# XuZhang1211/PVPUFormer

Hardware: AMD Instinct MI355X
Metric: 448x448 images/sec fwd+bwd, ViT-B VPUFormer (higher is better)
Workload: dtype bf16

## Files before the change

### include/vpu_hip.h

```cpp
#ifndef VPU_HIP_H
#define VPU_HIP_H
#include <stdint.h>

#ifdef __cplusplus
extern "C" {
#endif

#define VPU_BF16 0
#define VPU_F32 1

#define VPU_EPI_BIAS 1
#define VPU_EPI_PREACT 2
#define VPU_EPI_GELU 4
#define VPU_EPI_RELU 8
#define VPU_EPI_DGELU 16
#define VPU_EPI_DRELU 32
#define VPU_EPI_RESID 64
#define VPU_EPI_AFFINE 128
#define VPU_EPI_ACCUM 256
#define VPU_EPI_OUT_F32 512
#define VPU_EPI_SAVE_DGELU 1024
#define VPU_EPI_MULAUX 2048

typedef struct vpu_gemm_desc {
// ... 192 lines not shown
int vpu_groupnorm_nchunk(void);
int vpu_groupnorm_fwd(const void* x, const float* w, const float* b, void* y, float* mean, float* rstd, double* stats,
                      int32_t B, int64_t HW, int32_t C, float eps, int32_t gelu, int32_t dtype, void* stream);
int vpu_groupnorm_bwd(const void* dy, const void* x, const float* w, const float* b, const float* mean,
                      const float* rstd, void* dx, float* part, double* stats, int32_t B, int64_t HW, int32_t C,
                      int32_t gelu, int32_t dtype, void* stream);
int vpu_bilinear_cl_fwd(const void* in, int32_t ld_in, void* out, int32_t ld_out, int32_t B, int32_t h, int32_t w,
                        int32_t H, int32_t W, int32_t C, int32_t dtype, void* stream);
int vpu_bilinear_cl_bwd(const void* dout, int32_t ld_out, void* din, int32_t ld_in, int32_t B, int32_t h, int32_t w,
                        int32_t H, int32_t W, int32_t C, int32_t dtype, void* stream);
int vpu_upsum_relu(void* io, const void* const* z, const int32_t* h, const int32_t* w, int32_t n, int32_t B, int32_t H,
                   int32_t W, int32_t C, int32_t dtype, void* stream);
int vpu_head_grad_fused(const void* dfn, const void* y, const float* inv, const float* dout, const void* x, const float* w,
                        const float* mask, void* dx, float* part, float* part_b, int64_t rows, int64_t HW, int32_t C,
                        int32_t dtype, void* stream);
int vpu_gate_stats(const void* Q, const void* Kt, float* cg, int32_t* argq, float* sg, int32_t* argc, int32_t B,
                   int32_t nq, int32_t N, int32_t C, int32_t dtype, void* stream);
int vpu_gate_apply(const void* x, const float* cg, const float* sg, void* out, int32_t B, int32_t N, int32_t C,
                   int32_t dtype, void* stream);
int vpu_gate_bwd(const void* dout, const void* x, const float* cg, const int32_t* argq, const float* sg,
                 const int32_t* argc, void* dx, int32_t accum, void* dQ, void* dK, float* part, int32_t B, int32_t nq,
                 int32_t N, int32_t C, int32_t dtype, void* stream);
int vpu_gate_fwd_n(const void* const* Q, const void* const* K, const void* x, void* const* out, float* cg, int32_t* argq,
                   float* sg, int32_t* argc, int32_t n, int32_t B, int32_t nq, int32_t N, int32_t C, int32_t dtype, void* stream);
int vpu_gate_bwd_n(const void* const* dout, const void* x, const float* cg, const int32_t* argq, const float* sg,
                   const int32_t* argc, void* dx, int32_t accum, void* const* dQ, void* const* dK, float* part, int32_t n,
                   int32_t B, int32_t nq, int32_t N, int32_t C, int32_t dtype, void* stream);
int vpu_convseg_fwd(const void* x, const float* w, const float* bias, const float* mask, float* out, int64_t rows,
                    int64_t HW, int32_t C, int32_t dtype, void* stream);
int vpu_convseg_bwd_nblk(int64_t rows);
// ... 36 lines not shown
```

### pvpuformer_amd/_lib.py

```python
import ctypes as C
import os

_HERE = os.path.dirname(os.path.abspath(__file__))
LIB_PATH = os.path.join(_HERE, os.environ.get("VPU_LIB_FILE") or
                        ("libvpu_hip_diag.so" if os.environ.get("VPU_LIB_DIAG", "0") == "1" else "libvpu_hip.so"))

BF16, F32 = 0, 1

EPI_BIAS, EPI_PREACT, EPI_GELU, EPI_RELU, EPI_DGELU, EPI_DRELU = 1, 2, 4, 8, 16, 32
EPI_RESID, EPI_AFFINE, EPI_ACCUM, EPI_OUT_F32 = 64, 128, 256, 512
EPI_SAVE_DGELU, EPI_MULAUX = 1024, 2048


class GemmDesc(C.Structure):
    _fields_ = [
        ("A", C.c_void_p), ("B", C.c_void_p), ("C", C.c_void_p), ("bias", C.c_void_p), ("resid", C.c_void_p),
        ("aux", C.c_void_p), ("preact", C.c_void_p),
        ("M", C.c_int32), ("N", C.c_int32), ("K", C.c_int32),
        ("lda", C.c_int32), ("ldb", C.c_int32), ("ldc", C.c_int32), ("ldr", C.c_int32), ("ldaux", C.c_int32),
        ("batch", C.c_int32), ("inner", C.c_int32),
        ("sAo", C.c_int64), ("sAi", C.c_int64), ("sBo", C.c_int64), ("sBi", C.c_int64),
        ("sCo", C.c_int64), ("sCi", C.c_int64), ("sRo", C.c_int64), ("sRi", C.c_int64),
        ("transA", C.c_int32), ("transB", C.c_int32), ("dtype", C.c_int32), ("flags", C.c_int32),
        ("resid_period", C.c_int32),
# ... 92 lines not shown
    "vpu_patch_im2col_floor": [_P, _P, _P, _I, _I, _I, _I, _I, _I, _I, _P],
    "vpu_window_permute": [_P, _P, _I, _I, _I, _I, _I, _I, _P],
    "vpu_space_to_depth2_crop": [_P, _P, _I, _I, _I, _I, _I, _P],
    "vpu_pixel_shuffle2": [_P, _P, _P, _I, _I, _I, _I, _I, _I, _P],
    "vpu_pixel_shuffle2_gn_stats": [_P, _P, _P, _P, _I, _I, _I, _I, _I, _P],
    "vpu_groupnorm_apply": [_P, _P, _P, _P, _P, _P, _P, _I, _L, _I, _F, _I, _I, _P],
    "vpu_pixel_unshuffle2_nblk": [_I],
    "vpu_pixel_unshuffle2_sums": [_P, _P, _P, _I, _I, _I, _I, _I, _P],
    "vpu_groupnorm_nchunk": [],
    "vpu_groupnorm_fwd": [_P, _P, _P, _P, _P, _P, _P, _I, _L, _I, _F, _I, _I, _P],
    "vpu_groupnorm_bwd": [_P, _P, _P, _P, _P, _P, _P, _P, _P, _I, _L, _I, _I, _I, _P],
    "vpu_bilinear_cl_fwd": [_P, _I, _P, _I, _I, _I, _I, _I, _I, _I, _I, _P],
    "vpu_bilinear_cl_bwd": [_P, _I, _P, _I, _I, _I, _I, _I, _I, _I, _I, _P],
    "vpu_head_grad_fused": [_P, _P, _P, _P, _P, _P, _P, _P, _P, _P, _L, _L, _I, _I, _P],
    "vpu_upsum_relu": [_P, C.POINTER(C.c_void_p), C.POINTER(C.c_int32), C.POINTER(C.c_int32), _I, _I, _I, _I, _I, _I, _P],
    "vpu_gate_stats": [_P, _P, _P, _P, _P, _P, _I, _I, _I, _I, _I, _P],
    "vpu_gate_apply": [_P, _P, _P, _P, _I, _I, _I, _I, _P],
    "vpu_gate_bwd": [_P, _P, _P, _P, _P, _P, _P, _I, _P, _P, _P, _I, _I, _I, _I, _I, _P],
    "vpu_gate_fwd_n": [C.POINTER(C.c_void_p), C.POINTER(C.c_void_p), _P, C.POINTER(C.c_void_p), _P, _P, _P, _P, _I, _I, _I, _I, _I, _I, _P],
    "vpu_gate_bwd_n": [C.POINTER(C.c_void_p), _P, _P, _P, _P, _P, _P, _I, C.POINTER(C.c_void_p), C.POINTER(C.c_void_p), _P, _I, _I, _I,
                       _I, _I, _I, _P],
    "vpu_convseg_fwd": [_P, _P, _P, _P, _P, _L, _L, _I, _I, _P],
    "vpu_convseg_bwd_nblk": [_L],
    "vpu_convseg_bwd": [_P, _P, _P, _P, _P, _I, _P, _P, _L, _L, _I, _I, _P],
    "vpu_upsample_ac_fwd": [_P, _P, _L, _I, _I, _I, _I, _P],
    "vpu_upsample_ac_bwd": [_P, _P, _L, _I, _I, _I, _I, _P],
    "vpu_p2cl_fwd_bwd": [_P, _P, _P, _P, _P, _P, _F, _I, _I, _I, _I, _P],
    "vpu_p2cl_up_nband": [_I, _I],
    "vpu_p2cl_up_fwd_bwd": [_P, _P, _P, _P, _P, _P, _F, _I, _I, _I, _I, _I, _I, _P],
    "vpu_nfl_dice_scratch_doubles": [_I],
# ... 47 lines not shown
```

### pvpuformer_amd/csrc/spatial.hip

```cpp
#include <stdlib.h>
#include "vpu_common.h"
#include "interp_ac.h"
#include "../../include/vpu_hip.h"

#define DISPATCH_T(dtype, ...)                                   \
    if ((dtype) == VPU_BF16) { using T = bf16_t; __VA_ARGS__ }   \
    else if ((dtype) == VPU_F32) { using T = float; __VA_ARGS__ } \
    else { vpu_set_error("bad dtype"); return VPU_ERR_ARG; }
#define ST reinterpret_cast<hipStream_t>(stream)

namespace {

__constant__ float c_mean[3] = {0.485f, 0.456f, 0.406f};
__constant__ float c_std[3] = {0.229f, 0.224f, 0.225f};

template <typename T, bool NORM = true, bool VEC = true>
__global__ __launch_bounds__(256) void patch_im2col_kernel(const float* __restrict__ img4,
                                                           const float* __restrict__ disks, T* __restrict__ cols,
                                                           int B, int H, int W, int P, int wg) {
    const int gw = W / P, gh = H / P;
    const int K3 = 3 * P * P, K3P = (K3 + 7) / 8 * 8;
    const int Tn = gw * gh, KK = 2 * K3P, chunks = KK / 8;
    const int64_t total = (int64_t)B * Tn * chunks;
    const int nwx = gw / wg;
// ... 503 lines not shown
                const int64_t base = (int64_t)b * h * w;
                load8(in + (base + (int64_t)y0 * w + x0) * C + ck * 8, p);
                load8(in + (base + (int64_t)y0 * w + x1) * C + ck * 8, q);
                load8(in + (base + (int64_t)y1 * w + x0) * C + ck * 8, r);
                load8(in + (base + (int64_t)y1 * w + x1) * C + ck * 8, s);
#pragma unroll
                for (int j = 0; j < 8; ++j) o[j] += hy * (hx * p[j] + lx * q[j]) + ly * (hx * r[j] + lx * s[j]);
            }
#pragma unroll
        for (int j = 0; j < 8; ++j) o[j] = fmaxf(o[j], 0.f);
        store8(io + pix * C + ck * 8, o);
    }
}

template <typename T>
__global__ __launch_bounds__(256) void upsum_relu2_kernel(T* __restrict__ io, const UpsumArgs a, int B, int H, int W, int C) {
    const int chunks = C / 8, H2 = H >> 1, W2 = W >> 1;
    const int64_t total = (int64_t)B * H2 * W2 * chunks;
    for (int64_t i = (int64_t)blockIdx.x * 256 + threadIdx.x; i < total; i += (int64_t)gridDim.x * 256) {
        const int ck = (int)(i % chunks);
        const int64_t blk = i / chunks;
        const int X = 2 * (int)(blk % W2), Y = 2 * (int)((blk / W2) % H2), b = (int)(blk / ((int64_t)W2 * H2));
        float o[2][2][8];
#pragma unroll
        for (int dy = 0; dy < 2; ++dy)
#pragma unroll
            for (int dx = 0; dx < 2; ++dx) load8(io + (((int64_t)b * H + Y + dy) * W + X + dx) * C + ck * 8, o[dy][dx]);
#pragma unroll
        for (int m = 0; m < 3; ++m)
            if (m < a.n) {
                const int h = a.h[m], w = a.w[m];
                const T* __restrict__ in = reinterpret_cast<const T*>(a.z[m]) + (int64_t)b * h * w * C + ck * 8;
                int y0a, y1a, y0b, y1b, x0a, x1a, x0b, x1b;
                float lya, lyb, lxa, lxb;
                src_index_half(Y, (float)h / (float)H, h, y0a, y1a, lya);
                src_index_half(Y + 1, (float)h / (float)H, h, y0b, y1b, lyb);
                src_index_half(X, (float)w / (float)W, w, x0a, x1a, lxa);
                src_index_half(X + 1, (float)w / (float)W, w, x0b, x1b, lxb);
                const bool sy = y0b != y0a, sx = x0b != x0a;
                const int ry[3] = {y0a, y1a, y1b}, rx[3] = {x0a, x1a, x1b};
                float ha[3][8], hb[3][8];
#pragma unroll
                for (int r = 0; r < 3; ++r) {
                    if (r == 2 && !sy) continue;
                    float t0[8], t1[8], t2[8];
                    load8(in + ((int64_t)ry[r] * w + rx[0]) * C, t0);
                    load8(in + ((int64_t)ry[r] * w + rx[1]) * C, t1);
                    if (sx) load8(in + ((int64_t)ry[r] * w + rx[2]) * C, t2);
#pragma unroll
                    for (int j = 0; j < 8; ++j) {
                        ha[r][j] = (1.f - lxa) * t0[j] + lxa * t1[j];
                        const float u0 = sx ? t1[j] : t0[j], u1 = sx ? t2[j] : t1[j];
                        hb[r][j] = (1.f - lxb) * u0 + lxb * u1;
                    }
                }
#pragma unroll
                for (int j = 0; j < 8; ++j) {
                    o[0][0][j] += (1.f - lya) * ha[0][j] + lya * ha[1][j];
                    o[0][1][j] += (1.f - lya) * hb[0][j] + lya * hb[1][j];
                    const float a0 = sy ? ha[1][j] : ha[0][j], a1 = sy ? ha[2][j] : ha[1][j];
                    const float b0 = sy ? hb[1][j] : hb[0][j], b1 = sy ? hb[2][j] : hb[1][j];
                    o[1][0][j] += (1.f - lyb) * a0 + lyb * a1;
                    o[1][1][j] += (1.f - lyb) * b0 + lyb * b1;
                }
            }
#pragma unroll
        for (int dy = 0; dy < 2; ++dy)
#pragma unroll
            for (int dx = 0; dx < 2; ++dx) {
#pragma unroll
                for (int j = 0; j < 8; ++j) o[dy][dx][j] = fmaxf(o[dy][dx][j], 0.f);
                store8(io + (((int64_t)b * H + Y + dy) * W + X + dx) * C + ck * 8, o[dy][dx]);
            }
    }
}

template <typename T>
__global__ __launch_bounds__(256) void bilinear_cl_bwd_kernel(const T* __restrict__ dout, int ld_out,
                                                              T* __restrict__ din, int ld_in, int B, int h, int w, int H,
                                                              int W, int C) {
    const int chunks = C / 8;
    const float sh = (float)h / (float)H, sw = (float)w / (float)W;
    const float fh = (float)H / (float)h, fw = (float)W / (float)w;
    const int64_t total = (int64_t)B * h * w * chunks;
    for (int64_t i = (int64_t)blockIdx.x * 256 + threadIdx.x; i < total; i += (int64_t)gridDim.x * 256) {
        const int ck = (int)(i % chunks);
        const int64_t pix = i / chunks;
// ... 951 lines not shown
    a.n = n;
    for (int i = 0; i < 3; ++i) {
        a.z[i] = i < n ? z[i] : nullptr; a.h[i] = i < n ? h[i] : 1; a.w[i] = i < n ? w[i] : 1;
        if (i < n && (!z[i] || h[i] < 1 || w[i] < 1)) { vpu_set_error("upsum_relu: null / empty map"); return VPU_ERR_ARG; }
    }
    const int64_t total = (int64_t)B * H * W * (C / 8);
    bool quad = n > 0 && H % 2 == 0 && W % 2 == 0;
    for (int i = 0; i < n; ++i) quad = quad && H % h[i] == 0 && W % w[i] == 0 && H / h[i] >= 2 && W / w[i] >= 2;
    if (quad) {
        DISPATCH_T(dtype, upsum_relu2_kernel<T><<<vpu_grid_for(total / 4, 256, 16384), 256, 0, ST>>>((T*)io, a, B, H, W, C);)
    } else {
        DISPATCH_T(dtype, upsum_relu_kernel<T><<<vpu_grid_for(total, 256, 16384), 256, 0, ST>>>((T*)io, a, B, H, W, C);)
    }
    return vpu_check_launch("vpu_upsum_relu");
}
extern "C" int vpu_bilinear_cl_bwd(const void* dout, int32_t ld_out, void* din, int32_t ld_in, int32_t B, int32_t h,
                                   int32_t w, int32_t H, int32_t W, int32_t C, int32_t dtype, void* stream) {
    vpu_clear_stale_error();
    if (C % 8 || ld_in % 8 || ld_out % 8) { vpu_set_error("bilinear_cl_bwd: C, ld % 8"); return VPU_ERR_ARG; }
    const int64_t total = (int64_t)B * h * w * (C / 8);
    const int R = (h > 0 && w > 0 && H % h == 0 && W % w == 0 && H / h == W / w) ? H / h : 0;
    static const int split_min = [] { const char* e = vpu_lab_getenv("VPU_BILINEAR_SPLIT_R"); return e ? atoi(e) : 8; }();
    if ((R == 4 || R == 8) && R >= split_min && C == 256) {
        const unsigned g2 = (unsigned)(8 * ((((int64_t)B * h * w + 1) / 2 + 7) / 8));
        DISPATCH_T(dtype,
                   if (R == 4) bilinear_cl_bwd_int4_kernel<T, 4><<<g2, 256, 0, ST>>>((const T*)dout, ld_out, (T*)din, ld_in, B, h, w);
                   else bilinear_cl_bwd_int4_kernel<T, 8><<<g2, 256, 0, ST>>>((const T*)dout, ld_out, (T*)din, ld_in, B, h, w);)
        return vpu_check_launch("vpu_bilinear_cl_bwd");
    }
    if (R == 2 || R == 4 || R == 8) {
// ... 158 lines not shown
```

### pvpuformer_amd/engine.py

```python
import contextlib
import math
import os
from collections import OrderedDict
from types import SimpleNamespace

import numpy as np
import torch

from . import ops
from ._lib import (BF16, F32, EPI_BIAS, EPI_PREACT, EPI_GELU, EPI_RELU, EPI_DGELU, EPI_DRELU, EPI_RESID, EPI_AFFINE,
                   EPI_ACCUM, EPI_OUT_F32, EPI_SAVE_DGELU, EPI_MULAUX)


class Tape:
    __slots__ = ("fns", "out_grads", "done", "sim_low", "lane")

    def __init__(self):
        self.fns = []
        self.out_grads = [None, None, None]
        self.done = False
        self.sim_low = None
        self.lane = None

    def append(self, fn):
# ... 97 lines not shown
        self.wgrad_fill = 0.8
        hid = self.D * c["mlp_ratio"]
        blk = sum(((n + 255) // 256) * ((k + 127) // 128) for n, k in ((3 * self.D, self.D), (self.D, self.D), (hid, self.D), (self.D, hid)))
        pk = os.environ.get("VPU_WGRAD_PACK", "")
        k3 = ops.gemm_get_option("k3")
        k4_default = (k3 & 8) != 0
        self.pack_wgrad = pk == "1" or (pk != "0" and (blk < 0.95 * 256 or k4_default))
        self.k3_wgrad = (k3 & 1) != 0
        self.k4_wgrad = (k3 & 8) != 0
        self.wgrad_round = 256 if (self.k4_wgrad or not self.k3_wgrad) else 512
        self.wgrad_tn = 256 if self.k4_wgrad else 128
        self.unify_wgrad = True
        self.lazy_zero = True
        self.xattn_split = max(1, int(os.environ.get("VPU_XATTN_SPLIT", "1")))
        self.neck_lanes = int(os.environ.get("VPU_NECK_LANES", "0"))
        self._tok_stream = None
        self._in_lanes = False
        self.dist_colsum = True
        self._pack_seen, self._pack_total = {}, {}
        self._pending_reports, self._reporting = [], False
        self.group_tiles = 256
        self.split_wgrad = True
        self._wq = []
        self._csq = []
        self._gq = []
        self._gq_out = set()
        self._frozen = set()
        self._token_rows = 0
        self.grad_ready_hook = None
        self.report_lag = max(1, int(os.environ.get("VPU_DIST_REPORT_LAG", "2")))
# ... 983 lines not shown
        gf = self.G("head.fusion_conv.conv.weight")
        relu_done, ymask = [False], [[False] for _ in range(4)]
        ys, zs = [], []
        for i in range(4):
            f, s = feats[i]
            ys.append(self.linear(f, f"head.convs.{i}.conv.weight", f"head.convs.{i}.conv.bias", B * s * s, Cc, o[i],
                                  act="relu", pre_masked=ymask[i]))
        fused = Var(self._new(B * HW4, Cc))
        ops.gemm(ys[0].t, wf, fused.t, B * HW4, Cc, Cc, Cc, ldf, Cc, self.dt, flags=EPI_BIAS,
                 bias=self.Pm("head.fusion_conv.conv.bias"))
        for i in (1, 2, 3):
            s = feats[i][1]
            z = self._new(B * s * s, Cc)
            ops.gemm(ys[i].t, (wf[0], wf[1] + i * Cc), z, B * s * s, Cc, Cc, Cc, ldf, Cc, self.dt)
            zs.append((z, s, s))
        ops.upsum_relu(fused.t, zs, B, Hs, Hs, Cc, self.dt)
        if cx.training:
            def bwd_fusion():
                if fused.g is None:
                    return
                if relu_done[0]:
                    dt_ = fused.g
                else:
                    dt_ = self._new(B * HW4, Cc)
                    ops.act_bwd(fused.g, Cc, fused.t, Cc, dt_, Cc, B * HW4, Cc, 0, self.dt)
                self._wgrad(dt_, Cc, ys[0].t, Cc, gf, Cc, Cc, B * HW4, ldc=ldf, bias="head.fusion_conv.conv.bias")
                fuse_mask = self.dt == BF16
                mk = dict(flags=EPI_DRELU, ldaux=Cc) if fuse_mask else {}
                self._dgrad(dt_, Cc, wf, ldf, ys[0], B * HW4, Cc, Cc, **(dict(mk, aux=ys[0].t) if fuse_mask else {}))
                ymask[0][0] = fuse_mask
                for i in (1, 2, 3):
                    s = feats[i][1]
                    dz = self._new(B * s * s, Cc)
                    ops.bilinear_cl_bwd(dt_, Cc, dz, Cc, B, s, s, Hs, Hs, Cc, self.dt)
                    self._wgrad(dz, Cc, ys[i].t, Cc, (gf[0], gf[1] + i * Cc), Cc, Cc, B * s * s, ldc=ldf)
                    self._dgrad(dz, Cc, (wf[0], wf[1] + i * Cc), ldf, ys[i], B * s * s, Cc, Cc,
                                **(dict(mk, aux=ys[i].t) if fuse_mask else {}))
                    ymask[i][0] = fuse_mask
            self.tape.append(bwd_fusion)
        seg = self._new(B * HW4, dtype=torch.float32)
        ops.convseg_fwd(fused.t, self.Pm("head.conv_seg.weight"), self.Pm("head.conv_seg.bias"), drop_mask, seg,
                        B * HW4, HW4, Cc)
        dm = self.cfg["head_d_model"]
        query = self.mlp(q_out, "head.ffn_layer.lin1", "head.ffn_layer.lin2", B * nq, dm, 2 * dm, Cc, "relu")
        qn, fn = Var(torch.empty_like(query.t)), Var(torch.empty_like(fused.t))
        inv_q, inv_f = self._new(B * nq, dtype=torch.float32), self._new(B * HW4, dtype=torch.float32)
        ops.l2norm_fwd(query.t, qn.t, inv_q, B * nq, Cc)
        ops.l2norm_fwd(fused.t, fn.t, inv_f, B * HW4, Cc)
        sim = self._new(B, nq, HW4, dtype=torch.float32)
        ops.gemm(qn.t, fn.t, sim, nq, HW4, Cc, Cc, Cc, HW4, self.dt, flags=EPI_OUT_F32 | EPI_AFFINE, post_mul=0.5,
                 post_add=0.5, batch=B, inner=1, sA=(nq * Cc, 0), sB=(HW4 * Cc, 0), sC=(nq * HW4, 0))
        if cx.taps is not None:
            cx.taps["seg_lowres"] = seg.view(B, 1, Hs, Hs)
            cx.taps["sim_lowres"] = sim.view(B, nq, Hs, Hs)
            cx.taps["fused"] = fused.t
        inst = self._new(B, 1, H, W_, dtype=torch.float32)
        ops.upsample_ac_fwd(seg, inst, B, Hs, Hs, H, W_)
        aux = None
        self.sim_low = sim.view(B, nq, Hs, Hs)
        if materialize_aux:
            aux = self._new(B, nq, H, W_, dtype=torch.float32)
            ops.upsample_ac_fwd(sim, aux, B * nq, Hs, Hs, H, W_)
        tape.sim_low = self.sim_low
        if cx.training:
            def bwd_head():
                d_inst, d_aux, d_sim_low = tape.out_grads
                if d_aux is not None or d_sim_low is not None:
                    if d_sim_low is not None:
                        dsim = d_sim_low.view(B, nq, HW4)
                    else:
                        dsim = self._new(B, nq, HW4, dtype=torch.float32)
                        ops.upsample_ac_bwd(d_aux, dsim, B * nq, Hs, Hs, H, W_)
                    if self.dt == BF16:
                        dsim_t = self._new(B, nq, HW4)
                        ops.cast2d(dsim, HW4, dsim_t, HW4, B * nq, HW4)
                    else:
                        dsim_t = dsim
                    qn.g, fn.g = torch.empty_like(qn.t), torch.empty_like(fn.t)
                    ops.gemm(dsim_t, fn.t, qn.g, nq, Cc, HW4, HW4, Cc, Cc, self.dt, transB=True, alpha=0.5, batch=B,
                             inner=1, sA=(nq * HW4, 0), sB=(HW4 * Cc, 0), sC=(nq * Cc, 0))
                    ops.gemm(dsim_t, qn.t, fn.g, HW4, Cc, nq, HW4, Cc, Cc, self.dt, transA=True, transB=True, alpha=0.5,
# ... 314 lines not shown
```

### pvpuformer_amd/ops.py

```python
import ctypes as C

import torch

from . import _lib
from ._lib import (BF16, F32, EPI_BIAS, EPI_PREACT, EPI_GELU, EPI_RELU, EPI_DGELU, EPI_DRELU, EPI_RESID, EPI_AFFINE,
                   EPI_ACCUM, EPI_OUT_F32, EPI_SAVE_DGELU, EPI_MULAUX, GemmDesc)

TORCH_DTYPE = {BF16: torch.bfloat16, F32: torch.float32}


def code_of(t):
    if isinstance(t, tuple):
        t = t[0]
    if t.dtype == torch.bfloat16:
        return BF16
    if t.dtype == torch.float32:
        return F32
    raise TypeError(f"unsupported dtype {t.dtype}")


_raw_stream = getattr(torch._C, "_cuda_getCurrentRawStream", None)
_cur_device = getattr(torch._C, "_cuda_getDevice", None)


# ... 473 lines not shown
    _lib.call("vpu_bilinear_cl_fwd", ptr(inp), ld_in, ptr(out), ld_out, B, h, w, H, W, Cdim, dtype, _stream())


def bilinear_cl_bwd(dout, ld_out, din, ld_in, B, h, w, H, W, Cdim, dtype):
    _lib.call("vpu_bilinear_cl_bwd", ptr(dout), ld_out, ptr(din), ld_in, B, h, w, H, W, Cdim, dtype, _stream())


def upsum_relu(io, maps, B, H, W, Cdim, dtype):
    n = len(maps)
    zp = (C.c_void_p * 3)(*[ptr(m[0]) for m in maps])
    hs = (C.c_int32 * 3)(*[m[1] for m in maps])
    ws = (C.c_int32 * 3)(*[m[2] for m in maps])
    _lib.call("vpu_upsum_relu", ptr(io), zp, hs, ws, n, B, H, W, Cdim, dtype, _stream())


def gate_stats(Q, Kt, cg, argq, sg, argc, B, nq, N, Cdim):
    _lib.call("vpu_gate_stats", ptr(Q), ptr(Kt), ptr(cg), ptr(argq), ptr(sg), ptr(argc), B, nq, N, Cdim, code_of(Q),
              _stream())


def gate_apply(x, cg, sg, out, B, N, Cdim):
    _lib.call("vpu_gate_apply", ptr(x), ptr(cg), ptr(sg), ptr(out), B, N, Cdim, code_of(x), _stream())


def gate_bwd(dout, x, cg, argq, sg, argc, dx, accum, dQ, dK, part, B, nq, N, Cdim):
    _lib.call("vpu_gate_bwd", ptr(dout), ptr(x), ptr(cg), ptr(argq), ptr(sg), ptr(argc), ptr(dx), int(accum), ptr(dQ),
              ptr(dK), ptr(part), B, nq, N, Cdim, code_of(x), _stream())


def _ptr_array(ts):
# ... 81 lines not shown
```

Baseline: 994.9.

## Fuse head upsum/convseg/l2norm forward and stream head backward through one kernel

The forward path folds the multi-scale upsample-sum plus ReLU, the conv_seg projection and the L2 normalisation of fused features into one kernel. The backward path replaces the dsim cast, two batched GEMMs, l2norm backward and the conv_seg/ReLU gradient with a streaming MFMA kernel and a small finish kernel that reduces per-block query gradients. The goal is to cut repeated passes over the large HW×C feature map and the launch overhead of several kernels. In exchange it adds partial buffers for the query gradient, rounds dsim to bf16 before the GEMM, and only applies when C, nq and the map ratios fit the supported shapes.

```diff
diff --git a/include/vpu_hip.h b/include/vpu_hip.h
--- a/include/vpu_hip.h
+++ b/include/vpu_hip.h
@@ -230,6 +230,15 @@
 int vpu_head_grad_fused(const void* dfn, const void* y, const float* inv, const float* dout, const void* x, const float* w,
                         const float* mask, void* dx, float* part, float* part_b, int64_t rows, int64_t HW, int32_t C,
                         int32_t dtype, void* stream);
+int vpu_head_fuse_fwd(void* io, const void* const* z, const int32_t* h, const int32_t* w, int32_t n, int32_t B, int32_t H,
+                      int32_t W, int32_t C, const float* cw, const float* bias, const float* mask, float* seg, void* fn,
+                      float* inv, int32_t dtype, void* stream);
+int vpu_head_grad_stream_nblk(int64_t HW);
+int vpu_head_grad_stream(const float* dsim, const void* qn, const void* x, const float* inv, const float* dout, const float* w,
+                         const float* mask, void* dx, float* part, float* part_b, float* part_q, int32_t B, int64_t HW,
+                         int32_t nq, int32_t C, int32_t dtype, void* stream);
+int vpu_head_grad_finish(const float* part_q, const void* qn, const float* inv_q, void* dqn, void* dquery, int32_t B, int32_t nq,
+                         int32_t nblk, int32_t C, int32_t dtype, void* stream);
 int vpu_gate_stats(const void* Q, const void* Kt, float* cg, int32_t* argq, float* sg, int32_t* argc, int32_t B,
                    int32_t nq, int32_t N, int32_t C, int32_t dtype, void* stream);
 int vpu_gate_apply(const void* x, const float* cg, const float* sg, void* out, int32_t B, int32_t N, int32_t C,
diff --git a/pvpuformer_amd/_lib.py b/pvpuformer_amd/_lib.py
--- a/pvpuformer_amd/_lib.py
+++ b/pvpuformer_amd/_lib.py
@@ -130,6 +130,11 @@
     "vpu_bilinear_cl_bwd": [_P, _I, _P, _I, _I, _I, _I, _I, _I, _I, _I, _P],
     "vpu_head_grad_fused": [_P, _P, _P, _P, _P, _P, _P, _P, _P, _P, _L, _L, _I, _I, _P],
     "vpu_upsum_relu": [_P, C.POINTER(C.c_void_p), C.POINTER(C.c_int32), C.POINTER(C.c_int32), _I, _I, _I, _I, _I, _I, _P],
+    "vpu_head_fuse_fwd": [_P, C.POINTER(C.c_void_p), C.POINTER(C.c_int32), C.POINTER(C.c_int32), _I, _I, _I, _I, _I, _P, _P, _P, _P,
+                          _P, _P, _I, _P],
+    "vpu_head_grad_stream_nblk": [_L],
+    "vpu_head_grad_stream": [_P, _P, _P, _P, _P, _P, _P, _P, _P, _P, _P, _I, _L, _I, _I, _I, _P],
+    "vpu_head_grad_finish": [_P, _P, _P, _P, _P, _I, _I, _I, _I, _I, _P],
     "vpu_gate_stats": [_P, _P, _P, _P, _P, _P, _I, _I, _I, _I, _I, _P],
     "vpu_gate_apply": [_P, _P, _P, _P, _I, _I, _I, _I, _P],
     "vpu_gate_bwd": [_P, _P, _P, _P, _P, _P, _P, _I, _P, _P, _P, _I, _I, _I, _I, _I, _P],
diff --git a/pvpuformer_amd/csrc/headstream.hip b/pvpuformer_amd/csrc/headstream.hip
--- /dev/null
+++ b/pvpuformer_amd/csrc/headstream.hip
@@ -0,0 +1,346 @@
+#include "vpu_common.h"
+#include "../../include/vpu_hip.h"
+
+#define ST reinterpret_cast<hipStream_t>(stream)
+
+namespace {
+
+typedef __bf16 bf16x4_t __attribute__((ext_vector_type(4)));
+template <int VW> struct BVec;
+template <> struct BVec<8> { using type = bf16x8_t; };
+template <> struct BVec<4> { using type = bf16x4_t; };
+typedef unsigned hs_u32x4 __attribute__((ext_vector_type(4)));
+typedef unsigned hs_u32x2 __attribute__((ext_vector_type(2)));
+template <typename V> __device__ __forceinline__ void hs_pin(V& v) {
+    if constexpr (sizeof(V) == 16) {
+        hs_u32x4 t = __builtin_bit_cast(hs_u32x4, v);
+        asm volatile("" : "+v"(t));
+        v = __builtin_bit_cast(V, t);
+    } else {
+        hs_u32x2 t = __builtin_bit_cast(hs_u32x2, v);
+        asm volatile("" : "+v"(t));
+        v = __builtin_bit_cast(V, t);
+    }
+}
+
+constexpr int HS_ROWS = 64;
+#ifndef VPU_HS_BPI
+#define VPU_HS_BPI 40
+#endif
+constexpr int HS_BPI = VPU_HS_BPI;
+
+template <int C, int NT>
+struct HsCfg {
+    static constexpr int KS = NT > 2 ? 64 : 32;
+    static constexpr int VW = C >= 128 ? 8 : 4;
+    static constexpr int NG = C / (16 * VW);
+    static constexpr int CT = C / 64;
+    static constexpr int OFF_Q = 0;
+    static constexpr int OFF_Y = OFF_Q + C * KS * 2;
+    static constexpr int OFF_RS = OFF_Y + C * HS_ROWS * 2;
+    static constexpr int OFF_SR = OFF_RS + HS_ROWS * KS * 2;
+    static constexpr int BYTES = OFF_SR + 16 * NT * HS_ROWS * 2;
+};
+
+template <int RB> __device__ __forceinline__ int hs_idx(int row, int col) {
+    const int f = RB == 64 ? (row >> 1) & 7 : (row >> 2) & 3;
+    return row * RB + ((((col >> 3) ^ f) << 3) | (col & 7));
+}
+
+template <int C, int NT>
+__global__ __launch_bounds__(256, C <= 256 ? 2 : 1) void head_grad_stream_kernel(const float* __restrict__ dsim, const bf16_t* __restrict__ qn,
+                                                               const bf16_t* __restrict__ x, const float* __restrict__ inv,
+                                                               const float* __restrict__ dout, const float* __restrict__ w,
+                                                               const float* __restrict__ mask, bf16_t* __restrict__ dx,
+                                                               float* __restrict__ part, float* __restrict__ part_b,
+                                                               float* __restrict__ part_q, int HW, int nq, int bpi, int per) {
+    using Cfg = HsCfg<C, NT>;
+    constexpr int KS = Cfg::KS, VW = Cfg::VW, NG = Cfg::NG, CT = Cfg::CT, NSG = KS / 32;
+    using vec_t = typename BVec<VW>::type;
+    extern __shared__ __attribute__((aligned(16))) char lds[];
+    bf16_t* qT = reinterpret_cast<bf16_t*>(lds + Cfg::OFF_Q);
+    bf16_t* yT = reinterpret_cast<bf16_t*>(lds + Cfg::OFF_Y);
+    bf16_t* dRS = reinterpret_cast<bf16_t*>(lds + Cfg::OFF_RS);
+    bf16_t* dSR = reinterpret_cast<bf16_t*>(lds + Cfg::OFF_SR);
+    const int tid = threadIdx.x, lane = tid & 63, fr = lane & 15, fq = lane >> 4;
+    const int wave = __builtin_amdgcn_readfirstlane(tid >> 6);
+    const int b = blockIdx.x / bpi, kb = blockIdx.x - b * bpi;
+    const int r0 = kb * per, r1 = r0 + per < HW ? r0 + per : HW;
+    const float* __restrict__ ds_b = dsim + (int64_t)b * nq * HW;
+    const int64_t row_b = (int64_t)b * HW;
+    const bf16_t* __restrict__ x_b = x + row_b * C;
+    bf16_t* __restrict__ dx_b = dx + row_b * C;
+    const float* __restrict__ inv_b = inv + row_b;
+    const float* __restrict__ dout_b = dout + row_b;
+
+    for (int i = tid; i < KS * (C / 8); i += 256) {
+        const int s = i / (C / 8), c8 = (i - s * (C / 8)) * 8;
+        bf16x8_t v;
+#pragma unroll
+        for (int j = 0; j < 8; ++j) v[j] = (bf16_t)0.f;
+        if (s < nq) v = *reinterpret_cast<const bf16x8_t*>(qn + ((int64_t)b * nq + s) * C + c8);
+#pragma unroll
+        for (int j = 0; j < 8; ++j) {
+            const int c = c8 + j, g = c / (16 * VW), f = (c % (16 * VW)) / VW, t = c % VW;
+            qT[hs_idx<KS>((g * VW + t) * 16 + f, s)] = v[j];
+        }
+    }
+    const float* __restrict__ mask_b = mask ? mask + (int64_t)b * C : nullptr;
+    float dwa[NG][VW];
+#pragma unroll
+    for (int g = 0; g < NG; ++g)
+#pragma unroll
+        for (int t = 0; t < VW; ++t) dwa[g][t] = 0.f;
+    float dba = 0.f;
+    f32x4_t qacc[CT][NT];
+#pragma unroll
+    for (int m = 0; m < CT; ++m)
+#pragma unroll
+        for (int n = 0; n < NT; ++n) qacc[m][n] = f32x4_t{0.f, 0.f, 0.f, 0.f};
+
+    float pf[NSG][8];
+    const int rl = 16 * wave + 4 * fq;
+    auto fetch = [&](int rc) {
+        const int r = rc + lane, rv = r < r1 ? r : r1 - 1;
+#pragma unroll
+        for (int q = 0; q < NSG; ++q)
+#pragma unroll
+            for (int e = 0; e < 8; ++e) {
+                const int s = 8 * (wave + 4 * q) + e, sv = s < nq ? s : nq - 1;
+                const float v = (ds_b + (int64_t)sv * HW)[rv];
+                pf[q][e] = (s < nq && r < r1) ? v : 0.f;
+            }
+    };
+    fetch(r0);
+    for (int rc = r0; rc < r1; rc += HS_ROWS) {
+#pragma unroll
+        for (int q = 0; q < NSG; ++q) {
+            const int s8 = 8 * (wave + 4 * q);
+            bf16x8_t v;
+#pragma unroll
+            for (int e = 0; e < 8; ++e) v[e] = (bf16_t)pf[q][e];
+            *reinterpret_cast<bf16x8_t*>(dRS + hs_idx<KS>(lane, s8)) = v;
+            if (s8 < 16 * NT) {
+#pragma unroll
+                for (int e = 0; e < 8; ++e) dSR[hs_idx<HS_ROWS>(s8 + e, lane)] = v[e];
+            }
+        }
+        __syncthreads();
+        vec_t xp[NG][4];
+        float iv[4], dd[4];
+#pragma unroll
+        for (int i = 0; i < 4; ++i) {
+            const int rr = rc + rl + i, rv = rr < r1 ? rr : r1 - 1;
+            iv[i] = rr < r1 ? inv_b[rv] : 0.f;
+            dd[i] = rr < r1 ? dout_b[rv] : 0.f;
+#pragma unroll
+            for (int g = 0; g < NG; ++g) xp[g][i] = *reinterpret_cast<const vec_t*>(x_b + rv * C + 16 * VW * g + VW * fr);
+        }
+        if (rc + HS_ROWS < r1) fetch(rc + HS_ROWS);
+
+        int qoff = 0;
+        asm volatile("" : "+s"(qoff));
+        vec_t gp[NG][4];
+        float sdot[4] = {0.f, 0.f, 0.f, 0.f};
+#pragma unroll
+        for (int g = 0; g < NG; ++g) {
+            f32x4_t acc[VW];
+#pragma unroll
+            for (int t = 0; t < VW; ++t) acc[t] = f32x4_t{0.f, 0.f, 0.f, 0.f};
+#pragma unroll
+            for (int ks = 0; ks < NSG; ++ks) {
+                const bf16x8_t af = *reinterpret_cast<const bf16x8_t*>(dRS + hs_idx<KS>(16 * wave + fr, 32 * ks + 8 * fq));
+#pragma unroll
+                for (int t = 0; t < VW; ++t) {
+                    const bf16x8_t bq = *reinterpret_cast<const bf16x8_t*>(qT + qoff + hs_idx<KS>((g * VW + t) * 16 + fr, 32 * ks + 8 * fq));
+                    acc[t] = __builtin_amdgcn_mfma_f32_16x16x32_bf16(af, bq, acc[t], 0, 0, 0);
+                }
+            }
+#pragma unroll
+            for (int i = 0; i < 4; ++i)
+#pragma unroll
+                for (int t = 0; t < VW; ++t) {
+                    const bf16_t gv = (bf16_t)(0.5f * acc[t][i]);
+                    gp[g][i][t] = gv;
+                    const float yv = (float)(bf16_t)((float)xp[g][i][t] * iv[i]);
+                    sdot[i] += (float)gv * yv;
+                }
+        }
+#pragma unroll
+        for (int i = 0; i < 4; ++i)
+#pragma unroll
+            for (int o = 8; o > 0; o >>= 1) sdot[i] += __shfl_xor(sdot[i], o, 64);
+#pragma unroll
+        for (int i = 0; i < 4; ++i)
+            if (fr == 0) dba += dd[i];
+#pragma unroll
+        for (int g = 0; g < NG; ++g)
+#pragma unroll
+            for (int i = 0; i < 4; ++i) { hs_pin(xp[g][i]); hs_pin(gp[g][i]); }
+#pragma unroll
+        for (int g = 0; g < NG; ++g) {
+            float wv[VW], mk[VW];
+#pragma unroll
+            for (int t = 0; t < VW; t += 4) {
+                const int c = qoff + 16 * VW * g + VW * fr + t;
+                const f32x4_t a = *reinterpret_cast<const f32x4_t*>(w + c);
+                f32x4_t m = f32x4_t{1.f, 1.f, 1.f, 1.f};
+                if (mask_b) m = *reinterpret_cast<const f32x4_t*>(mask_b + c);
+#pragma unroll
+                for (int u = 0; u < 4; ++u) { wv[t + u] = a[u]; mk[t + u] = m[u]; }
+            }
+            bf16x4_t yq[VW];
+#pragma unroll
+            for (int i = 0; i < 4; ++i) {
+                vec_t ov;
+#pragma unroll
+                for (int t = 0; t < VW; ++t) {
+                    const float xv = (float)xp[g][i][t];
+                    const bf16_t yb = (bf16_t)(xv * iv[i]);
+                    yq[t][i] = yb;
+                    dwa[g][t] += dd[i] * xv * mk[t];
+                    const float tt = iv[i] * ((float)gp[g][i][t] - (float)yb * sdot[i]) + dd[i] * wv[t] * mk[t];
+                    ov[t] = (bf16_t)(xv > 0.f ? tt : 0.f);
+                }
+                if (rc + rl + i < r1) *reinterpret_cast<vec_t*>(dx_b + (rc + rl + i) * C + 16 * VW * g + VW * fr) = ov;
+            }
+#pragma unroll
+            for (int t = 0; t < VW; ++t) *reinterpret_cast<bf16x4_t*>(yT + hs_idx<HS_ROWS>(16 * VW * g + VW * fr + t, rl)) = yq[t];
+        }
+        __syncthreads();
+
+#pragma unroll
+        for (int ks = 0; ks < HS_ROWS / 32; ++ks) {
+            bf16x8_t af[CT], bs[NT];
+#pragma unroll
+            for (int m = 0; m < CT; ++m)
+                af[m] = *reinterpret_cast<const bf16x8_t*>(yT + hs_idx<HS_ROWS>(16 * (wave * CT + m) + fr, 32 * ks + 8 * fq));
+#pragma unroll
+            for (int n = 0; n < NT; ++n) bs[n] = *reinterpret_cast<const bf16x8_t*>(dSR + hs_idx<HS_ROWS>(16 * n + fr, 32 * ks + 8 * fq));
+#pragma unroll
+            for (int m = 0; m < CT; ++m)
+#pragma unroll
+                for (int n = 0; n < NT; ++n) qacc[m][n] = __builtin_amdgcn_mfma_f32_16x16x32_bf16(af[m], bs[n], qacc[m][n], 0, 0, 0);
+        }
+        __syncthreads();
+    }
+
+#pragma unroll
+    for (int m = 0; m < CT; ++m)
+#pragma unroll
+        for (int n = 0; n < NT; ++n) {
+            const int s = 16 * n + fr;
+            if (s < nq)
+                *reinterpret_cast<f32x4_t*>(part_q + ((int64_t)blockIdx.x * nq + s) * C + 16 * (wave * CT + m) + 4 * fq) = qacc[m][n];
+        }
+    float* red = reinterpret_cast<float*>(lds + Cfg::OFF_Y);
+#pragma unroll
+    for (int g = 0; g < NG; ++g)
+#pragma unroll
+        for (int t = 0; t < VW; ++t) {
+            float v = dwa[g][t];
+            v += __shfl_xor(v, 16, 64);
+            v += __shfl_xor(v, 32, 64);
+            if (fq == 0) red[wave * C + 16 * VW * g + VW * fr + t] = v;
+        }
+    dba = wave_sum(dba);
+    if (lane == 0) red[4 * C + wave] = dba;
+    __syncthreads();
+    for (int c = tid; c < C; c += 256) part[(int64_t)blockIdx.x * C + c] = red[c] + red[C + c] + red[2 * C + c] + red[3 * C + c];
+    if (tid == 0) part_b[blockIdx.x] = red[4 * C] + red[4 * C + 1] + red[4 * C + 2] + red[4 * C + 3];
+}
+
+__global__ __launch_bounds__(256) void head_grad_finish_kernel(const float* __restrict__ part_q, const bf16_t* __restrict__ qn,
+                                                               const float* __restrict__ inv_q, bf16_t* __restrict__ dqn,
+                                                               bf16_t* __restrict__ dquery, int nq, int bpi, int C) {
+    __shared__ float red[16];
+    const int row = blockIdx.x, b = row / nq, s = row - b * nq;
+    const float* __restrict__ p = part_q + ((int64_t)b * bpi * nq + s) * C;
+    const int64_t step = (int64_t)nq * C;
+    float g[2] = {0.f, 0.f}, y[2] = {0.f, 0.f};
+    float dot = 0.f;
+#pragma unroll
+    for (int k = 0; k < 2; ++k) {
+        const int c = threadIdx.x + 256 * k;
+        if (c < C) {
+            float t = 0.f;
+#pragma unroll 8
+            for (int j = 0; j < bpi; ++j) t += p[j * step + c];
+            const bf16_t gv = (bf16_t)(0.5f * t);
+            dqn[(int64_t)row * C + c] = gv;
+            g[k] = (float)gv;
+            y[k] = (float)qn[(int64_t)row * C + c];
+            dot += g[k] * y[k];
+        }
+    }
+    dot = block_sum(dot, red);
+    const float iv = inv_q[row];
+#pragma unroll
+    for (int k = 0; k < 2; ++k) {
+        const int c = threadIdx.x + 256 * k;
+        if (c < C) dquery[(int64_t)row * C + c] = (bf16_t)(iv * (g[k] - y[k] * dot));
+    }
+}
+
+inline int hs_per(int64_t HW) {
+    const int64_t chunks = (HW + HS_ROWS - 1) / HS_ROWS;
+    return (int)((chunks + HS_BPI - 1) / HS_BPI) * HS_ROWS;
+}
+
+template <int C, int NT>
+int hs_launch(const float* dsim, const void* qn, const void* x, const float* inv, const float* dout, const float* w,
+              const float* mask, void* dx, float* part, float* part_b, float* part_q, int B, int HW, int nq, int bpi, int per,
+              void* stream) {
+    static VpuDevOnce once;
+    constexpr int bytes = HsCfg<C, NT>::BYTES;
+    const auto kern = head_grad_stream_kernel<C, NT>;
+    if (auto todo = once.pending()) { VPU_SET_LDS(bytes, kern); }
+    kern<<<(unsigned)(B * bpi), 256, bytes, ST>>>(
+        dsim, (const bf16_t*)qn, (const bf16_t*)x, inv, dout, w, mask, (bf16_t*)dx, part, part_b, part_q, HW, nq, bpi, per);
+    return vpu_check_launch("vpu_head_grad_stream");
+}
+
+}
+
+extern "C" int vpu_head_grad_stream_nblk(int64_t HW) {
+    vpu_clear_stale_error();
+    if (HW < 1) return 1;
+    const int per = hs_per(HW);
+    return (int)((HW + per - 1) / per);
+}
+
+extern "C" int vpu_head_grad_stream(const float* dsim, const void* qn, const void* x, const float* inv, const float* dout,
+                                    const float* w, const float* mask, void* dx, float* part, float* part_b, float* part_q,
+                                    int32_t B, int64_t HW, int32_t nq, int32_t C, int32_t dtype, void* stream) {
+    vpu_clear_stale_error();
+    auto a16 = [](const void* p) { return reinterpret_cast<uintptr_t>(p) % 16 == 0; };
+    if (dtype != VPU_BF16 || !(C == 64 || C == 128 || C == 256 || C == 512) || nq < 1 || nq > 64 || B < 1 || HW < 1 ||
+        HW > (1 << 21) || (int64_t)B * vpu_head_grad_stream_nblk(HW) > (1 << 30) || !dsim || !qn || !x || !inv || !dout || !w ||
+        !dx || !part || !part_b || !part_q || !a16(qn) || !a16(x) || !a16(dx) || !a16(part_q) || !a16(w) || !a16(mask)) {
+        vpu_set_error("head_grad_stream: bf16, C in {64,128,256,512}, 1 <= nq <= 64, non-null 16-byte aligned operands");
+        return VPU_ERR_ARG;
+    }
+    const int per = hs_per(HW), bpi = (int)((HW + per - 1) / per), nt = (nq + 15) / 16;
+#define VPU_HS_NT(C_)                                                                                                         \
+    switch (nt) {                                                                                                             \
+        case 1: return hs_launch<C_, 1>(dsim, qn, x, inv, dout, w, mask, dx, part, part_b, part_q, B, (int)HW, nq, bpi, per, stream); \
+        case 2: return hs_launch<C_, 2>(dsim, qn, x, inv, dout, w, mask, dx, part, part_b, part_q, B, (int)HW, nq, bpi, per, stream); \
+        case 3: return hs_launch<C_, 3>(dsim, qn, x, inv, dout, w, mask, dx, part, part_b, part_q, B, (int)HW, nq, bpi, per, stream); \
+        default: return hs_launch<C_, 4>(dsim, qn, x, inv, dout, w, mask, dx, part, part_b, part_q, B, (int)HW, nq, bpi, per, stream); \
+    }
+    if (C == 64) { VPU_HS_NT(64) } else if (C == 128) { VPU_HS_NT(128) } else if (C == 256) { VPU_HS_NT(256) } else { VPU_HS_NT(512) }
+#undef VPU_HS_NT
+}
+
+extern "C" int vpu_head_grad_finish(const float* part_q, const void* qn, const float* inv_q, void* dqn, void* dquery, int32_t B,
+                                    int32_t nq, int32_t bpi, int32_t C, int32_t dtype, void* stream) {
+    vpu_clear_stale_error();
+    if (dtype != VPU_BF16 || !(C == 64 || C == 128 || C == 256 || C == 512) || nq < 1 || B < 1 || bpi < 1 || !part_q || !qn ||
+        !inv_q || !dqn || !dquery) {
+        vpu_set_error("head_grad_finish: bf16, C in {64,128,256,512}, non-null operands");
+        return VPU_ERR_ARG;
+    }
+    head_grad_finish_kernel<<<(unsigned)(B * nq), 256, 0, ST>>>(part_q, (const bf16_t*)qn, inv_q, (bf16_t*)dqn, (bf16_t*)dquery, nq,
+                                                               bpi, C);
+    return vpu_check_launch("vpu_head_grad_finish");
+}
diff --git a/pvpuformer_amd/csrc/spatial.hip b/pvpuformer_amd/csrc/spatial.hip
--- a/pvpuformer_amd/csrc/spatial.hip
+++ b/pvpuformer_amd/csrc/spatial.hip
@@ -541,6 +541,52 @@
 }
 
 template <typename T>
+__device__ __forceinline__ void upsum_quad(const T* __restrict__ io, const UpsumArgs& a, int b, int Y, int X, int H, int W, int C,
+                                           int ck, float (&o)[2][2][8]) {
+#pragma unroll
+    for (int dy = 0; dy < 2; ++dy)
+#pragma unroll
+        for (int dx = 0; dx < 2; ++dx) load8(io + (((int64_t)b * H + Y + dy) * W + X + dx) * C + ck * 8, o[dy][dx]);
+#pragma unroll
+    for (int m = 0; m < 3; ++m)
+        if (m < a.n) {
+            const int h = a.h[m], w = a.w[m];
+            const T* __restrict__ in = reinterpret_cast<const T*>(a.z[m]) + (int64_t)b * h * w * C + ck * 8;
+            int y0a, y1a, y0b, y1b, x0a, x1a, x0b, x1b;
+            float lya, lyb, lxa, lxb;
+            src_index_half(Y, (float)h / (float)H, h, y0a, y1a, lya);
+            src_index_half(Y + 1, (float)h / (float)H, h, y0b, y1b, lyb);
+            src_index_half(X, (float)w / (float)W, w, x0a, x1a, lxa);
+            src_index_half(X + 1, (float)w / (float)W, w, x0b, x1b, lxb);
+            const bool sy = y0b != y0a, sx = x0b != x0a;
+            const int ry[3] = {y0a, y1a, y1b}, rx[3] = {x0a, x1a, x1b};
+            float ha[3][8], hb[3][8];
+#pragma unroll
+            for (int r = 0; r < 3; ++r) {
+                if (r == 2 && !sy) continue;
+                float t0[8], t1[8], t2[8];
+                load8(in + ((int64_t)ry[r] * w + rx[0]) * C, t0);
+                load8(in + ((int64_t)ry[r] * w + rx[1]) * C, t1);
+                if (sx) load8(in + ((int64_t)ry[r] * w + rx[2]) * C, t2);
+#pragma unroll
+                for (int j = 0; j < 8; ++j) {
+                    ha[r][j] = (1.f - lxa) * t0[j] + lxa * t1[j];
+                    const float u0 = sx ? t1[j] : t0[j], u1 = sx ? t2[j] : t1[j];
+                    hb[r][j] = (1.f - lxb) * u0 + lxb * u1;
+                }
+            }
+#pragma unroll
+            for (int j = 0; j < 8; ++j) {
+                o[0][0][j] += (1.f - lya) * ha[0][j] + lya * ha[1][j];
+                o[0][1][j] += (1.f - lya) * hb[0][j] + lya * hb[1][j];
+                const float a0 = sy ? ha[1][j] : ha[0][j], a1 = sy ? ha[2][j] : ha[1][j];
+                const float b0 = sy ? hb[1][j] : hb[0][j], b1 = sy ? hb[2][j] : hb[1][j];
+                o[1][0][j] += (1.f - lyb) * a0 + lyb * a1;
+                o[1][1][j] += (1.f - lyb) * b0 + lyb * b1;
+            }
+        }
+}
+template <typename T>
 __global__ __launch_bounds__(256) void upsum_relu2_kernel(T* __restrict__ io, const UpsumArgs a, int B, int H, int W, int C) {
     const int chunks = C / 8, H2 = H >> 1, W2 = W >> 1;
     const int64_t total = (int64_t)B * H2 * W2 * chunks;
@@ -549,48 +595,7 @@
         const int64_t blk = i / chunks;
         const int X = 2 * (int)(blk % W2), Y = 2 * (int)((blk / W2) % H2), b = (int)(blk / ((int64_t)W2 * H2));
         float o[2][2][8];
-#pragma unroll
-        for (int dy = 0; dy < 2; ++dy)
-#pragma unroll
-            for (int dx = 0; dx < 2; ++dx) load8(io + (((int64_t)b * H + Y + dy) * W + X + dx) * C + ck * 8, o[dy][dx]);
-#pragma unroll
-        for (int m = 0; m < 3; ++m)
-            if (m < a.n) {
-                const int h = a.h[m], w = a.w[m];
-                const T* __restrict__ in = reinterpret_cast<const T*>(a.z[m]) + (int64_t)b * h * w * C + ck * 8;
-                int y0a, y1a, y0b, y1b, x0a, x1a, x0b, x1b;
-                float lya, lyb, lxa, lxb;
-                src_index_half(Y, (float)h / (float)H, h, y0a, y1a, lya);
-                src_index_half(Y + 1, (float)h / (float)H, h, y0b, y1b, lyb);
-                src_index_half(X, (float)w / (float)W, w, x0a, x1a, lxa);
-                src_index_half(X + 1, (float)w / (float)W, w, x0b, x1b, lxb);
-                const bool sy = y0b != y0a, sx = x0b != x0a;
-                const int ry[3] = {y0a, y1a, y1b}, rx[3] = {x0a, x1a, x1b};
-                float ha[3][8], hb[3][8];
-#pragma unroll
-                for (int r = 0; r < 3; ++r) {
-                    if (r == 2 && !sy) continue;
-                    float t0[8], t1[8], t2[8];
-                    load8(in + ((int64_t)ry[r] * w + rx[0]) * C, t0);
-                    load8(in + ((int64_t)ry[r] * w + rx[1]) * C, t1);
-                    if (sx) load8(in + ((int64_t)ry[r] * w + rx[2]) * C, t2);
-#pragma unroll
-                    for (int j = 0; j < 8; ++j) {
-                        ha[r][j] = (1.f - lxa) * t0[j] + lxa * t1[j];
-                        const float u0 = sx ? t1[j] : t0[j], u1 = sx ? t2[j] : t1[j];
-                        hb[r][j] = (1.f - lxb) * u0 + lxb * u1;
-                    }
-                }
-#pragma unroll
-                for (int j = 0; j < 8; ++j) {
-                    o[0][0][j] += (1.f - lya) * ha[0][j] + lya * ha[1][j];
-                    o[0][1][j] += (1.f - lya) * hb[0][j] + lya * hb[1][j];
-                    const float a0 = sy ? ha[1][j] : ha[0][j], a1 = sy ? ha[2][j] : ha[1][j];
-                    const float b0 = sy ? hb[1][j] : hb[0][j], b1 = sy ? hb[2][j] : hb[1][j];
-                    o[1][0][j] += (1.f - lyb) * a0 + lyb * a1;
-                    o[1][1][j] += (1.f - lyb) * b0 + lyb * b1;
-                }
-            }
+        upsum_quad(io, a, b, Y, X, H, W, C, ck, o);
 #pragma unroll
         for (int dy = 0; dy < 2; ++dy)
 #pragma unroll
@@ -598,6 +603,55 @@
 #pragma unroll
                 for (int j = 0; j < 8; ++j) o[dy][dx][j] = fmaxf(o[dy][dx][j], 0.f);
                 store8(io + (((int64_t)b * H + Y + dy) * W + X + dx) * C + ck * 8, o[dy][dx]);
+            }
+    }
+}
+
+__global__ __launch_bounds__(256, 3) void head_fuse_fwd_kernel(bf16_t* __restrict__ io, const UpsumArgs a, const float* __restrict__ w,
+                                                            const float* __restrict__ bias, const float* __restrict__ mask,
+                                                            float* __restrict__ seg, bf16_t* __restrict__ fn,
+                                                            float* __restrict__ inv, int B, int H, int W, int C) {
+    const int chunks = C / 8, H2 = H >> 1, W2 = W >> 1;
+    const int64_t total = (int64_t)B * H2 * W2 * chunks;
+    const float b0 = bias[0];
+    int cur_b = -1;
+    float wm[8];
+    for (int64_t i = (int64_t)blockIdx.x * 256 + threadIdx.x; i < total; i += (int64_t)gridDim.x * 256) {
+        const int ck = (int)(i % chunks);
+        const int64_t blk = i / chunks;
+        const int X = 2 * (int)(blk % W2), Y = 2 * (int)((blk / W2) % H2), b = (int)(blk / ((int64_t)W2 * H2));
+        if (b != cur_b) {
+            cur_b = b;
+            load8(w + ck * 8, wm);
+            if (mask) {
+                float mk[8];
+                load8(mask + (int64_t)b * C + ck * 8, mk);
+#pragma unroll
+                for (int j = 0; j < 8; ++j) wm[j] *= mk[j];
+            }
+        }
+        float o[2][2][8];
+        upsum_quad(io, a, b, Y, X, H, W, C, ck, o);
+#pragma unroll
+        for (int dy = 0; dy < 2; ++dy)
+#pragma unroll
+            for (int dx = 0; dx < 2; ++dx) {
+                const int64_t row = ((int64_t)b * H + Y + dy) * W + X + dx;
+                float v[8];
+#pragma unroll
+                for (int j = 0; j < 8; ++j) v[j] = (float)(bf16_t)fmaxf(o[dy][dx][j], 0.f);
+                store8(io + row * C + ck * 8, v);
+                float s = 0.f, q = 0.f;
+#pragma unroll
+                for (int j = 0; j < 8; ++j) s += v[j] * wm[j];
+#pragma unroll
+                for (int j = 0; j < 8; ++j) q += v[j] * v[j];
+                for (int x = chunks >> 1; x > 0; x >>= 1) { s += __shfl_xor(s, x, 64); q += __shfl_xor(q, x, 64); }
+                const float iv = 1.0f / fmaxf(sqrtf(q), 1e-12f);
+                if (ck == 0) { seg[row] = s + b0; inv[row] = iv; }
+#pragma unroll
+                for (int j = 0; j < 8; ++j) v[j] *= iv;
+                store8(fn + row * C + ck * 8, v);
             }
     }
 }
@@ -1579,6 +1633,30 @@
     }
     return vpu_check_launch("vpu_upsum_relu");
 }
+extern "C" int vpu_head_fuse_fwd(void* io, const void* const* z, const int32_t* h, const int32_t* w, int32_t n, int32_t B,
+                                 int32_t H, int32_t W, int32_t C, const float* cw, const float* bias, const float* mask,
+                                 float* seg, void* fn, float* inv, int32_t dtype, void* stream) {
+    vpu_clear_stale_error();
+    auto a16 = [](const void* p) { return reinterpret_cast<uintptr_t>(p) % 16 == 0; };
+    bool ok = dtype == VPU_BF16 && (C == 64 || C == 128 || C == 256 || C == 512) && io && z && h && w && n >= 1 && n <= 3 &&
+              B >= 1 && H >= 2 && W >= 2 && H % 2 == 0 && W % 2 == 0 && cw && bias && seg && fn && inv && a16(io) && a16(fn) &&
+              (reinterpret_cast<uintptr_t>(cw) | reinterpret_cast<uintptr_t>(mask)) % 32 == 0;
+    UpsumArgs a;
+    a.n = n;
+    for (int i = 0; i < 3; ++i) {
+        const bool in = ok && i < n;
+        a.z[i] = in ? z[i] : nullptr; a.h[i] = in ? h[i] : 1; a.w[i] = in ? w[i] : 1;
+        if (in) ok = z[i] && a16(z[i]) && h[i] >= 1 && w[i] >= 1 && H % h[i] == 0 && W % w[i] == 0 && H / h[i] >= 2 && W / w[i] >= 2;
+    }
+    if (!ok) {
+        vpu_set_error("head_fuse_fwd: bf16, C in {64,128,256,512}, 1 <= n <= 3 maps at integer ratios >= 2, even H / W, aligned non-null operands");
+        return VPU_ERR_ARG;
+    }
+    const int64_t total = (int64_t)B * H * W * (C / 8);
+    head_fuse_fwd_kernel<<<vpu_grid_for(total / 4, 256, 16384), 256, 0, ST>>>((bf16_t*)io, a, cw, bias, mask, seg, (bf16_t*)fn,
+                                                                              inv, B, H, W, C);
+    return vpu_check_launch("vpu_head_fuse_fwd");
+}
 extern "C" int vpu_bilinear_cl_bwd(const void* dout, int32_t ld_out, void* din, int32_t ld_in, int32_t B, int32_t h,
                                    int32_t w, int32_t H, int32_t W, int32_t C, int32_t dtype, void* stream) {
     vpu_clear_stale_error();
diff --git a/pvpuformer_amd/engine.py b/pvpuformer_amd/engine.py
--- a/pvpuformer_amd/engine.py
+++ b/pvpuformer_amd/engine.py
@@ -135,6 +135,7 @@
         self.lazy_zero = True
         self.xattn_split = max(1, int(os.environ.get("VPU_XATTN_SPLIT", "1")))
         self.neck_lanes = int(os.environ.get("VPU_NECK_LANES", "0"))
+        self.head_stream = int(os.environ.get("VPU_HEAD_STREAM", "1"))
         self._tok_stream = None
         self._in_lanes = False
         self.dist_colsum = True
@@ -1148,7 +1149,14 @@
             z = self._new(B * s * s, Cc)
             ops.gemm(ys[i].t, (wf[0], wf[1] + i * Cc), z, B * s * s, Cc, Cc, Cc, ldf, Cc, self.dt)
             zs.append((z, s, s))
-        ops.upsum_relu(fused.t, zs, B, Hs, Hs, Cc, self.dt)
+        seg = self._new(B * HW4, dtype=torch.float32)
+        fn, inv_f = Var(torch.empty_like(fused.t)), self._new(B * HW4, dtype=torch.float32)
+        fuse_fwd = self.head_stream in (1, 2) and ops.head_fuse_ok(zs, Hs, Hs, Cc, self.dt)
+        if fuse_fwd:
+            ops.head_fuse_fwd(fused.t, zs, self.Pm("head.conv_seg.weight"), self.Pm("head.conv_seg.bias"), drop_mask, seg,
+                              fn.t, inv_f, B, Hs, Hs, Cc)
+        else:
+            ops.upsum_relu(fused.t, zs, B, Hs, Hs, Cc, self.dt)
         if cx.training:
             def bwd_fusion():
                 if fused.g is None:
@@ -1172,15 +1180,15 @@
                                 **(dict(mk, aux=ys[i].t) if fuse_mask else {}))
                     ymask[i][0] = fuse_mask
             self.tape.append(bwd_fusion)
-        seg = self._new(B * HW4, dtype=torch.float32)
-        ops.convseg_fwd(fused.t, self.Pm("head.conv_seg.weight"), self.Pm("head.conv_seg.bias"), drop_mask, seg,
-                        B * HW4, HW4, Cc)
+        if not fuse_fwd:
+            ops.convseg_fwd(fused.t, self.Pm("head.conv_seg.weight"), self.Pm("head.conv_seg.bias"), drop_mask, seg,
+                            B * HW4, HW4, Cc)
         dm = self.cfg["head_d_model"]
         query = self.mlp(q_out, "head.ffn_layer.lin1", "head.ffn_layer.lin2", B * nq, dm, 2 * dm, Cc, "relu")
-        qn, fn = Var(torch.empty_like(query.t)), Var(torch.empty_like(fused.t))
-        inv_q, inv_f = self._new(B * nq, dtype=torch.float32), self._new(B * HW4, dtype=torch.float32)
+        qn, inv_q = Var(torch.empty_like(query.t)), self._new(B * nq, dtype=torch.float32)
         ops.l2norm_fwd(query.t, qn.t, inv_q, B * nq, Cc)
-        ops.l2norm_fwd(fused.t, fn.t, inv_f, B * HW4, Cc)
+        if not fuse_fwd:
+            ops.l2norm_fwd(fused.t, fn.t, inv_f, B * HW4, Cc)
         sim = self._new(B, nq, HW4, dtype=torch.float32)
         ops.gemm(qn.t, fn.t, sim, nq, HW4, Cc, Cc, Cc, HW4, self.dt, flags=EPI_OUT_F32 | EPI_AFFINE, post_mul=0.5,
                  post_add=0.5, batch=B, inner=1, sA=(nq * Cc, 0), sB=(HW4 * Cc, 0), sC=(nq * HW4, 0))
@@ -1199,6 +1207,23 @@
         if cx.training:
             def bwd_head():
                 d_inst, d_aux, d_sim_low = tape.out_grads
+                if (self.head_stream in (1, 3) and d_sim_low is not None and d_inst is not None and d_aux is None and
+                        self.dt == BF16 and Cc in ops.HEAD_STREAM_C and nq <= ops.HEAD_STREAM_NQ):
+                    dseg = self._new(B * HW4, dtype=torch.float32)
+                    ops.upsample_ac_bwd(d_inst, dseg, B, Hs, Hs, H, W_)
+                    nbi = ops.head_grad_stream_nblk(HW4)
+                    nb = B * nbi
+                    part, part_b = self._new(nb, Cc, dtype=torch.float32), self._new(nb, dtype=torch.float32)
+                    part_q = self._new(nb, nq, Cc, dtype=torch.float32)
+                    fused.g = torch.empty_like(fused.t)
+                    ops.head_grad_stream(d_sim_low.view(B, nq, HW4), qn.t, fused.t, inv_f, dseg, self.Pm("head.conv_seg.weight"),
+                                         drop_mask, fused.g, part, part_b, part_q, B, HW4, nq, Cc)
+                    qn.g, query.g = torch.empty_like(qn.t), torch.empty_like(query.t)
+                    ops.head_grad_finish(part_q, qn.t, inv_q, qn.g, query.g, B, nq, nbi, Cc)
+                    relu_done[0] = True
+                    self._csq.append((part, self.G("head.conv_seg.weight"), nb, Cc))
+                    self._csq.append((part_b, self.G("head.conv_seg.bias"), nb, 1))
+                    return
                 if d_aux is not None or d_sim_low is not None:
                     if d_sim_low is not None:
                         dsim = d_sim_low.view(B, nq, HW4)
diff --git a/pvpuformer_amd/ops.py b/pvpuformer_amd/ops.py
--- a/pvpuformer_amd/ops.py
+++ b/pvpuformer_amd/ops.py
@@ -511,6 +511,38 @@
     _lib.call("vpu_upsum_relu", ptr(io), zp, hs, ws, n, B, H, W, Cdim, dtype, _stream())
 
 
+HEAD_STREAM_C = (64, 128, 256, 512)
+HEAD_STREAM_NQ = 64
+
+
+def head_fuse_ok(maps, H, W, Cdim, dtype):
+    return (dtype == _lib.BF16 and Cdim in HEAD_STREAM_C and 1 <= len(maps) <= 3 and H % 2 == 0 and W % 2 == 0 and
+            all(H % h == 0 and W % w == 0 and H // h >= 2 and W // w >= 2 for _, h, w in maps))
+
+
+def head_fuse_fwd(io, maps, w, bias, mask, seg, fn, inv, B, H, W, Cdim):
+    n = len(maps)
+    zp = (C.c_void_p * 3)(*[ptr(m[0]) for m in maps])
+    hs = (C.c_int32 * 3)(*[m[1] for m in maps])
+    ws = (C.c_int32 * 3)(*[m[2] for m in maps])
+    _lib.call("vpu_head_fuse_fwd", ptr(io), zp, hs, ws, n, B, H, W, Cdim, ptr(w), ptr(bias), ptr(mask), ptr(seg), ptr(fn),
+              ptr(inv), code_of(io), _stream())
+
+
+def head_grad_stream_nblk(HW):
+    return _lib.load().vpu_head_grad_stream_nblk(HW)
+
+
+def head_grad_stream(dsim, qn, x, inv, dout, w, mask, dx, part, part_b, part_q, B, HW, nq, Cdim):
+    _lib.call("vpu_head_grad_stream", ptr(dsim), ptr(qn), ptr(x), ptr(inv), ptr(dout), ptr(w), ptr(mask), ptr(dx), ptr(part),
+              ptr(part_b), ptr(part_q), B, HW, nq, Cdim, code_of(x), _stream())
+
+
+def head_grad_finish(part_q, qn, inv_q, dqn, dquery, B, nq, nblk, Cdim):
+    _lib.call("vpu_head_grad_finish", ptr(part_q), ptr(qn), ptr(inv_q), ptr(dqn), ptr(dquery), B, nq, nblk, Cdim, code_of(qn),
+              _stream())
+
+
 def gate_stats(Q, Kt, cg, argq, sg, argc, B, nq, N, Cdim):
     _lib.call("vpu_gate_stats", ptr(Q), ptr(Kt), ptr(cg), ptr(argq), ptr(sg), ptr(argc), B, nq, N, Cdim, code_of(Q),
               _stream())
```

Result: no change. 1001 (median of 6 runs) (+0.6%).
